# WU-CVGL/SIU3R

Hardware: AMD Instinct MI355X
Metric: image-pairs/sec @2x512^2 (SIU3R network forward incl. panoptic post-process) (higher is better)
Workload: dtype bf16x3 (fp32 activations, bf16 MFMA with hi/lo operand split; meets the 1e-3 parity bar)

## Files before the change

### siu3r_amd/csrc/gemm.hip

```cpp
#include <stdlib.h>

#include "common.h"
#include "gemm_epilogue.h"

int siu3r_gemm_dma_launch(const siu3r_gemm_params& p, int ni, void* stream);
int siu3r_gemm_dma_x3_launch(const siu3r_gemm_params& p, void* stream);
int siu3r_gemm_dma_mode(const siu3r_gemm_params& p);
int siu3r_gemm_dma_x3_mode(const siu3r_gemm_params& p);
int siu3r_gemm_pp_mode(const siu3r_gemm_params& p);
void siu3r_gemm_pp_name(const siu3r_gemm_params& p, int cfg, char* buf, int n);
int siu3r_gemm_pp_launch(const siu3r_gemm_params& p, int cfg, void* stream);
int siu3r_gemm_skinny_launch(const siu3r_gemm_params& p, void* stream);
int siu3r_gemm_skinny_path(const siu3r_gemm_params& p);
int siu3r_gemm_dma_kspl();
bool siu3r_gemm_pp_a_x3_ok(const siu3r_gemm_params& p);
bool siu3r_gemm_pp_c_x3_ok(const siu3r_gemm_params& p, int cfg);
static const bool g_disable_dma = getenv("SIU3R_GEMM_NO_DMA") != nullptr;
static const int g_narrow_max = getenv("SIU3R_GEMM_NARROW_MAX") ? atoi(getenv("SIU3R_GEMM_NARROW_MAX")) : 0x7fffffff;

namespace {

constexpr int BM = 128, BK = 64;
constexpr int A_TILE_BYTES = BM * BK * 2;

__device__ __forceinline__ int lds_off(int row, int chunk) {
  return row * 128 + ((chunk ^ ((row >> 1) & 7)) << 4);
}

template <int A_F32, int SPLIT, int NI>
struct Regs {
  float4 ra0[A_F32 ? 4 : 1], ra1[A_F32 ? 4 : 1];
  uint4 rab[A_F32 ? 1 : 4];
  uint4 rwh[2 * NI], rwl[SPLIT ? 2 * NI : 1];
};

template <int A_F32, int SPLIT, int NI, bool LNF = false>
__global__ __launch_bounds__(256) void gemm_kernel(const siu3r_gemm_params p) {
  constexpr int BN = 64 * NI;
  constexpr int B_TILE_BYTES = BN * BK * 2;
// ... 362 lines not shown
  const Cand& c = kCands[best];
  pl.tile_cfg = c.cfg;
  pl.bm = c.bm;
  pl.bn = c.bn;
  pl.splitk = best_s;
  pl.skinny_rows = best_skinny;
  if (c.cfg > 0 && best_skinny > 0) {
    siu3r_gemm_params q = p;
    q.m_main = p.m - best_skinny;
    pl.skinny_path = siu3r_gemm_skinny_path(q);
  }
  if (c.cfg < 0) {
    const int64_t tiles128 = (int64_t)((p.m + BM - 1) / BM) * ((p.n + 127) / 128) * Z;
    const bool narrow = (p.n <= 64) || (tiles128 < g_narrow_max && p.n > 64) || p.w_x3 != nullptr;
    pl.bn = narrow ? 64 : 128;
    if (!narrow || dma_mode < 0) pl.splitk = 1;
  }
  if (pl.splitk > 1) {
    const int64_t tiles = (int64_t)((p.m - pl.skinny_rows + pl.bm - 1) / pl.bm) * ((p.n + pl.bn - 1) / pl.bn) * Z;
    pl.ws_floats = tiles * pl.splitk * pl.bm * pl.bn;
    pl.counters = (int32_t)tiles;
  }
  auto tf = [](bool b) { return b ? "true" : "false"; };
  if (c.cfg > 0) {
    siu3r_gemm_pp_name(p, c.cfg, pl.kernel, sizeof(pl.kernel));
  } else if (x3 && dma_mode >= 0 && pl.bn == 64) {
    snprintf(pl.kernel, sizeof(pl.kernel), "siu3r_gemm_dma::gemm_dma_x3_kernel<%d, %s, %d, %s>", dma_mode, tf(dma_mode == 1 && p.relu_in), siu3r_gemm_dma_kspl(), tf(dma_mode == 0 && p.ln_stats));
  } else if (!x3 && !p.w_lo && dma_mode >= 0) {
    snprintf(pl.kernel, sizeof(pl.kernel), "siu3r_gemm_dma::gemm_dma_kernel<%d, %d, %s, %d, %s>", pl.bn / 64, dma_mode, tf(dma_mode == 1 && p.relu_in), siu3r_gemm_dma_kspl(), tf(dma_mode == 0 && p.ln_stats));
  } else {
    snprintf(pl.kernel, sizeof(pl.kernel), "gemm_kernel<%d, %d, %d%s>", p.a_dtype == SIU3R_F32 ? 1 : 0, p.w_lo ? 1 : 0, pl.bn / 64, p.ln_stats ? ", true" : "");
  }
}
}

static int validate_gemm(const siu3r_gemm_params& p) {
  SIU3R_CHECK(p.a && p.w_hi && (p.c || p.c_x3), "siu3r_gemm: null operand pointer");
  SIU3R_CHECK(p.m > 0 && p.n > 0 && p.k > 0, "siu3r_gemm: empty problem (m=%d n=%d k=%d)", p.m, p.n, p.k);
  SIU3R_CHECK(p.kpad % BK == 0 && p.kpad >= p.k, "siu3r_gemm: kpad=%d must be a multiple of 64 and >= k=%d", p.kpad, p.k);
  SIU3R_CHECK(p.a_dtype == SIU3R_BF16 || p.a_dtype == SIU3R_F32, "siu3r_gemm: bad a_dtype %d", p.a_dtype);
  SIU3R_CHECK(p.c_dtype == SIU3R_BF16 || p.c_dtype == SIU3R_F32, "siu3r_gemm: bad c_dtype %d", p.c_dtype);
  SIU3R_CHECK(!(p.w_lo && p.a_dtype != SIU3R_F32), "siu3r_gemm: bf16x3 mode needs fp32 activations");
  SIU3R_CHECK(p.a_mode >= 0 && p.a_mode <= 2, "siu3r_gemm: bad a_mode %d", p.a_mode);
  if (p.a_mode != 0) SIU3R_CHECK(p.oh > 0 && p.ow > 0 && p.ih > 0 && p.iw > 0 && (p.a_mode == 2 || (p.cin > 0 && p.kh > 0 && p.kw > 0 && p.stride > 0)),
                                 "siu3r_gemm: conv geometry must be positive (ih=%d iw=%d cin=%d kh=%d kw=%d stride=%d oh=%d ow=%d)", p.ih, p.iw, p.cin, p.kh, p.kw, p.stride, p.oh, p.ow);
  if (p.a_mode == 0) {
    SIU3R_CHECK(p.k % 8 == 0 && p.lda % 8 == 0, "siu3r_gemm: dense A needs k %% 8 == 0 and lda %% 8 == 0 (k=%d lda=%ld)", p.k, (long)p.lda);
  } else if (p.a_mode == 1) {
    SIU3R_CHECK(p.cin % 8 == 0 || (p.cin % 4 == 0 && p.w_x3 && p.a_dtype == SIU3R_F32 && !p.relu_in && !g_disable_dma),
                "siu3r_gemm: conv gather needs cin %% 8 == 0 (cin %% 4 == 0 for fp32 activations with w_x3) (cin=%d)", p.cin);
    SIU3R_CHECK(p.k == p.kh * p.kw * p.cin, "siu3r_gemm: conv k=%d != kh*kw*cin", p.k);
    SIU3R_CHECK(p.m % (p.oh * p.ow) == 0, "siu3r_gemm: conv m=%d not a multiple of oh*ow", p.m);
  } else {
    SIU3R_CHECK(p.a_dtype == SIU3R_F32 && p.k == 768 && p.ih == p.oh * 16 && p.iw == p.ow * 16,
                "siu3r_gemm: patchify mode needs fp32 NCHW input, k=768, H,W multiples of 16");
  }
  if (p.out_mode == 1) SIU3R_CHECK(p.n == p.up * p.up * p.cout && p.m % (p.ih * p.iw) == 0 && p.cout % 8 == 0, "siu3r_gemm: bad conv-transpose geometry (cout %% 8 == 0 required)");
  if (p.rope_cos) SIU3R_CHECK(p.rope_sin && p.rope_pos && p.rope_ncols % 64 == 0 && p.rope_ncols <= p.n && p.act == 0 && p.out_mode == 0,
                              "siu3r_gemm: bad RoPE epilogue arguments");
  if (p.up_src) SIU3R_CHECK(p.a_mode == 1 && p.out_mode == 0 && p.oh % 2 == 0 && p.ow % 2 == 0, "siu3r_gemm: up_src needs conv mode with even output size");
  if (p.ln_stats)
    SIU3R_CHECK(p.ln_c1 && p.ln_c2 && !p.bias && p.a_mode == 0 && p.ln_tiles == (p.k + 63) / 64 && p.ln_tiles <= 16 && !p.relu_in,
                "siu3r_gemm: folded LayerNorm needs c1/c2, no bias, dense A and ln_tiles == ceil(k/64) <= 16 (k=%d, ln_tiles=%d)", p.k, p.ln_tiles);
  if (p.stats_out) SIU3R_CHECK(p.out_mode == 0 && !p.up_src, "siu3r_gemm: stats_out needs a plain row-major output");
  if (p.c_aux) SIU3R_CHECK(p.out_mode == 0, "siu3r_gemm: c_aux needs a plain row-major output");
  if (p.splitk > 1)
    SIU3R_CHECK(p.sk_ws && p.sk_cnt && p.splitk <= 64 && p.splitk <= p.kpad / 64, "siu3r_gemm: split-K needs a workspace, zeroed counters and splitk <= kpad / 64 (splitk=%d)", p.splitk);
  SIU3R_CHECK(p.tile_cfg >= -1 && p.tile_cfg <= 3, "siu3r_gemm: bad tile_cfg %d", p.tile_cfg);
  if (p.bmod > 0) SIU3R_CHECK(p.batch > 0 && p.batch % p.bmod == 0, "siu3r_gemm: batch %d is not a multiple of bmod %d", p.batch, p.bmod);
  return 0;
}

extern "C" int siu3r_gemm_plan(const siu3r_gemm_params* pp, siu3r_gemm_plan_t* out) {
  SIU3R_CHECK(pp && out, "siu3r_gemm_plan: null argument");
  if (int rc = validate_gemm(*pp)) return rc;
  plan(*pp, *out);
  out->a_x3_ok = out->tile_cfg > 0 && siu3r_gemm_pp_a_x3_ok(*pp);
  out->c_x3_ok = out->tile_cfg > 0 && siu3r_gemm_pp_c_x3_ok(*pp, out->tile_cfg);
  return 0;
}

extern "C" int siu3r_gemm(const siu3r_gemm_params* pp, void* stream) {
  const siu3r_gemm_params& p = *pp;
  if (int rc = validate_gemm(p)) return rc;
  siu3r_gemm_plan_t pl;
  plan(p, pl);
  hipStream_t s = (hipStream_t)stream;
  SIU3R_CHECK(!p.a_x3 || (pl.tile_cfg > 0 && siu3r_gemm_pp_a_x3_ok(p)), "siu3r_gemm: a_x3 (pre-split A planes) needs a ping-pong plan, bf16x3 weights, dense A, "
              "k == kpad and lda / batch strides %% 32 == 0 (this block runs %s): query siu3r_gemm_plan_t.a_x3_ok first", pl.kernel);
  SIU3R_CHECK(!p.c_x3 || (pl.tile_cfg > 0 && siu3r_gemm_pp_c_x3_ok(p, pl.tile_cfg)), "siu3r_gemm: c_x3 (output planes) needs a ping-pong plan and the plain fp32 "
              "row-major output form with n %% 64 == 0, ldc / batch strides %% 32 == 0 (this block runs %s): query siu3r_gemm_plan_t.c_x3_ok first", pl.kernel);
  SIU3R_CHECK(p.c || p.c_x3, "siu3r_gemm: null output");
  siu3r_gemm_params q = p;
  q.splitk = pl.splitk;
  if (pl.splitk > 1) SIU3R_CHECK(p.sk_ws && p.sk_cnt && p.sk_ws_floats >= pl.ws_floats && p.sk_cnt_n >= pl.counters,
                                 "siu3r_gemm: split-K workspace too small (%ld floats / %d counters needed)", (long)pl.ws_floats, pl.counters);
  SIU3R_CHECK(!(p.splitk > 1 && pl.splitk != p.splitk), "siu3r_gemm: splitk=%d was requested but %s cannot split K for this problem (it would run %d slice(s)); "
              "request 0 / 1 or another tile_cfg", p.splitk, pl.kernel, pl.splitk);
  if (pl.tile_cfg > 0) {
    q.m_main = pl.skinny_rows > 0 ? p.m - pl.skinny_rows : 0;
    if (!(pl.skinny_rows > 0 && q.m_main == 0)) {
      const int rc = siu3r_gemm_pp_launch(q, pl.tile_cfg, stream);
      if (rc) return rc;
    }
    if (pl.skinny_rows > 0 && siu3r_gemm_skinny_path(q) != 1) {
      q.splitk = 0;
      return siu3r_gemm_skinny_launch(q, stream);
    }
    return 0;
  }
  return pl.bn == 64 ? launch<1>(q, s) : launch<2>(q, s);
}
```

### siu3r_amd/csrc/gemm_dma.hip

```cpp
#include <stdlib.h>

#include "common.h"
#include "gemm_epilogue.h"

namespace siu3r_gemm_dma {

constexpr int BM = 128, BK = 64, STAGES = 3;
#ifndef SIU3R_GEMM_PD_WIDE
#define SIU3R_GEMM_PD_WIDE 2
#endif
constexpr int A_TILE_BYTES = BM * BK * 2;
constexpr unsigned OOB = 0xffffff00u;
constexpr int RSRC_FLAGS = 0x00020000;

typedef __attribute__((address_space(3))) void* lds_ptr;
typedef __attribute__((ext_vector_type(4))) unsigned int u32x4;
typedef __attribute__((ext_vector_type(2))) short i16x2;

template <int NI, int MODE, bool RELU, int KSPL, bool LNF = false>
__global__ __launch_bounds__(256 * KSPL, NI == 1 ? 2 * KSPL : 1) void gemm_dma_kernel(const siu3r_gemm_params p) {
#if __HIP_DEVICE_COMPILE__
  constexpr int BN = 64 * NI;
  constexpr int B_TILE_BYTES = BN * BK * 2;
  constexpr int STAGE_BYTES = A_TILE_BYTES + B_TILE_BYTES;
// ... 337 lines not shown
  for (int kt = 0; kt < nkt; kt += 2) {
    tile_body(kt, st, fA0, fB0, fA1, fB1);
    st = (st + 1 == STAGES) ? 0 : st + 1;
    if (kt + 1 < nkt) {
      tile_body(kt + 1, st, fA1, fB1, fA0, fB0);
      st = (st + 1 == STAGES) ? 0 : st + 1;
    }
  }
#undef SIU3R_WAIT_FRAGS
  asm volatile("s_waitcnt vmcnt(0)" ::: "memory");
  stamp(4);

  if (dbg & 1) { if (acc[0][0][0] == 123.456f) ((float*)p.c)[0] = 1.f; return; }
  siu3r_epi::run<NI, KSPL, LNF>(p, acc, smem, tile_m, tile_n, z, t);
  if (trace && t == 0) {
    trace[6] = __builtin_readcyclecounter();
    asm volatile("s_waitcnt vmcnt(0)" ::: "memory");
    trace[7] = __builtin_readcyclecounter();
  }
#endif
}


template <int MODE, bool RELU, int KSPL, bool LNF = false>
__global__ __launch_bounds__(256 * KSPL, 2 * KSPL) void gemm_dma_x3_kernel(const siu3r_gemm_params p) {
#if __HIP_DEVICE_COMPILE__
  constexpr int BN = 64, BKE = 32;
  constexpr int B_TILE_BYTES = BN * 128;
  constexpr int STAGE_BYTES = A_TILE_BYTES + B_TILE_BYTES;
  constexpr int A_DMA = 4 / KSPL, W_DMA = 2 / KSPL, LP = A_DMA + W_DMA;
  constexpr int KSW = 2 / KSPL;
  static_assert(STAGES * STAGE_BYTES >= siu3r_epi::staging_bytes<1, KSPL>(), "epilogue staging must fit the ring");
  __shared__ __attribute__((aligned(128))) unsigned char smem[STAGES * STAGE_BYTES];

  const int t = threadIdx.x;
  const int lane = t & 63;
  const int wave = __builtin_amdgcn_readfirstlane(t >> 6);
  const int khalf = wave >> 2, wq = wave & 3;
  const int wm = wq >> 1, wn = wq & 1;
  const int l31 = lane & 31, lh = lane >> 5;

  const int M = p.m, N = p.n, K = p.k, kpad = p.kpad;
  const int tiles_m = (M + BM - 1) / BM, tiles_n = (N + BN - 1) / BN;
  const int xcd = (blockIdx.x + blockIdx.z) & 7, li = blockIdx.x >> 3;
  const int map_gx = p.map_gx;
  const int ry = xcd / map_gx, rx = xcd - ry * map_gx;
  const int lm = li / p.map_rn, ln = li - lm * p.map_rn;
  const int tile_m = ry * p.map_rm + lm, tile_n = rx * p.map_rn + ln;
  if (lm >= p.map_rm || tile_m >= tiles_m || tile_n >= tiles_n) return;
// ... 125 lines not shown
    unsigned char* dst = smem + stage * STAGE_BYTES + A_TILE_BYTES + (wave * W_DMA + i) * 1024;
    __builtin_amdgcn_raw_ptr_buffer_load_lds(rW, (lds_ptr)dst, 16, w_voff[i], (kbase + kt) * 128, 0, 0);
  };
  auto issue = [&](int kt, int stage) {
#pragma unroll
    for (int i = 0; i < A_DMA; ++i) issue_a(kt, stage, i);
#pragma unroll
    for (int i = 0; i < W_DMA; ++i) issue_w(kt, stage, i);
    if (MODE == 1) cursor_advance();
    if (MODE == 2) state_advance();
  };

  f32x16 acc[2][1];
#pragma unroll
  for (int i = 0; i < 2; ++i)
#pragma unroll
    for (int r = 0; r < 16; ++r) acc[i][0][r] = 0.f;

  const unsigned int lds_base = (unsigned int)(size_t)(__attribute__((address_space(3))) unsigned char*)smem;
  unsigned int offA[2], offB;
#pragma unroll
  for (int i = 0; i < 2; ++i) {
    const int row = wm * 64 + i * 32 + l31;
    offA[i] = row * 128 + ((((lh << 1)) ^ ((row >> 1) & 7)) << 4);
  }
  {
    const int row = wn * 32 + l31;
    offB = A_TILE_BYTES + row * 128 + ((lh ^ ((row >> 1) & 7)) << 4);
  }
  struct Frag {
    u32x4 a[2][2], bh, bl;
  };
  auto read_sub = [&](unsigned int sbase, int ks, Frag& f) {
#pragma unroll
    for (int i = 0; i < 2; ++i) {
      const unsigned int ad = (sbase + offA[i]) ^ (ks << 6);
      asm volatile("ds_read_b128 %0, %1" : "=v"(f.a[i][0]) : "v"(ad) : "memory");
      asm volatile("ds_read_b128 %0, %1 offset:0" : "=v"(f.a[i][1]) : "v"(ad ^ 16u) : "memory");
    }
    const unsigned int adb = (sbase + offB) ^ (ks << 5);
    asm volatile("ds_read_b128 %0, %1" : "=v"(f.bh) : "v"(adb) : "memory");
    asm volatile("ds_read_b128 %0, %1" : "=v"(f.bl) : "v"(adb ^ 64u) : "memory");
  };
  auto issue_tile_reads = [&](int stage, Frag (&f)[KSW]) {
    const unsigned int sbase = lds_base + stage * STAGE_BYTES;
#pragma unroll
    for (int j = 0; j < KSW; ++j) read_sub(sbase, khalf * KSW + j, f[j]);
  };
  auto split8 = [&](const u32x4& v0, const u32x4& v1, bf16x8& hi, bf16x8& lo) {
    unsigned int w[8] = {v0[0], v0[1], v0[2], v0[3], v1[0], v1[1], v1[2], v1[3]};
    union { u32x4 u; bf16x8 h; } H, L;
#pragma unroll
    for (int q = 0; q < 4; ++q) {
      unsigned int x0 = w[2 * q], x1 = w[2 * q + 1];
      if (RELU) {
        x0 = (x0 & 0x80000000u) ? 0u : x0;
        x1 = (x1 & 0x80000000u) ? 0u : x1;
      }
      const unsigned int h0 = x0 & 0xffff0000u, h1 = x1 & 0xffff0000u;
      const float l0 = __uint_as_float(x0) - __uint_as_float(h0), l1 = __uint_as_float(x1) - __uint_as_float(h1);
      H.u[q] = __builtin_amdgcn_perm(x1, x0, 0x07060302u);
// ... 17 lines not shown
#pragma unroll
        for (int i = 0; i < A_DMA; ++i) issue_a(kt_next, stage_next, i);
#pragma unroll
        for (int i = 0; i < W_DMA; ++i) issue_w(kt_next, stage_next, i);
      }
      if (j == KSW - 1 && kt + 1 < nkt) {
        if (kt_next >= 0) {
          if (LP == 6) asm volatile("s_waitcnt vmcnt(6)" ::: "memory");
          else asm volatile("s_waitcnt vmcnt(3)" ::: "memory");
        } else {
          asm volatile("s_waitcnt vmcnt(0)" ::: "memory");
        }
        __builtin_amdgcn_s_barrier();
        asm volatile("" ::: "memory");
        issue_tile_reads(stage_read, nf);
      }
      __builtin_amdgcn_sched_barrier(0);
      union { u32x4 u; bf16x8 h; } bh, bl;
      bh.u = f[j].bh;
      bl.u = f[j].bl;
#pragma unroll
      for (int i = 0; i < 2; ++i) {
        bf16x8 ah, al;
        split8(f[j].a[i][0], f[j].a[i][1], ah, al);
        acc[i][0] = __builtin_amdgcn_mfma_f32_32x32x16_bf16(al, bh.h, acc[i][0], 0, 0, 0);
        acc[i][0] = __builtin_amdgcn_mfma_f32_32x32x16_bf16(ah, bl.h, acc[i][0], 0, 0, 0);
        acc[i][0] = __builtin_amdgcn_mfma_f32_32x32x16_bf16(ah, bh.h, acc[i][0], 0, 0, 0);
      }
      if (KSW == 2 && kt_next >= 0 && j == 0) {
#pragma unroll
        for (int i = 0; i < A_DMA; ++i) issue_a(kt_next, stage_next, i);
#pragma unroll
        for (int i = 0; i < W_DMA; ++i) issue_w(kt_next, stage_next, i);
      }
      __builtin_amdgcn_sched_barrier(0);
    }
    if (MODE == 1 && kt_next >= 0) cursor_advance();
    if (MODE == 2 && kt_next >= 0) state_advance();
  };

  for (int q = 0; q < kbase; ++q) {
    if (MODE == 1) cursor_advance();
    if (MODE == 2) state_advance();
  }
  issue(0, 0);
  if (nkt > 1) issue(1, 1);
  if (nkt > 1) {
    if (LP == 6) asm volatile("s_waitcnt vmcnt(6)" ::: "memory");
    else asm volatile("s_waitcnt vmcnt(3)" ::: "memory");
  } else {
    asm volatile("s_waitcnt vmcnt(0)" ::: "memory");
  }
  __builtin_amdgcn_s_barrier();
  asm volatile("" ::: "memory");
  Frag f0[KSW], f1[KSW];
  issue_tile_reads(0, f0);
  int st = 0;
  for (int kt = 0; kt < nkt; kt += 2) {
    tile_body(kt, st, f0, f1);
    st = (st + 1 == STAGES) ? 0 : st + 1;
    if (kt + 1 < nkt) {
      tile_body(kt + 1, st, f1, f0);
      st = (st + 1 == STAGES) ? 0 : st + 1;
    }
  }
#undef SIU3R_X3_WAIT
  asm volatile("s_waitcnt vmcnt(0)" ::: "memory");
  siu3r_epi::run<1, KSPL, LNF>(p, acc, smem, tile_m, tile_n, z, t);
#endif
}

}

int siu3r_gemm_dma_mode(const siu3r_gemm_params& p) {
  const int64_t lim = 0xfffff000ll;
  if (p.w_lo || p.a_dtype != SIU3R_BF16 || p.a_mode == 2) return -1;
  if ((int64_t)p.n * p.kpad * 2 >= lim) return -1;
  if (p.a_mode == 0) return (((int64_t)(p.m - 1) * p.lda + p.k) * 2 >= lim || p.relu_in) ? -1 : 0;
  const int64_t img = (int64_t)(p.m / (p.oh * p.ow)) * p.ih * p.iw * p.cin * 2 + (int64_t)(p.pad * p.iw + p.pad) * p.cin * 2;
  if (img >= lim) return -1;
  const int mode = (p.cin % 64 == 0 && p.kh * p.kw <= 32 && p.kpad == p.k) ? 1 : 2;
  return (mode == 2 && p.relu_in) ? -1 : mode;
}
int siu3r_gemm_dma_x3_mode(const siu3r_gemm_params& p) {
  const int64_t lim = 0xfffff000ll;
  if (!p.w_x3 || p.a_dtype != SIU3R_F32 || (int64_t)p.n * p.kpad * 4 >= lim) return -1;
  if (p.a_mode == 0) return (((int64_t)(p.m - 1) * p.lda + p.k) * 4 >= lim || p.relu_in) ? -1 : 0;
  if (p.a_mode != 1) return -1;
  const int64_t img = (int64_t)(p.m / (p.oh * p.ow)) * p.ih * p.iw * p.cin * 4 + (int64_t)(p.pad * p.iw + p.pad) * p.cin * 4;
  if (img >= lim || p.cin % 4 != 0) return -1;
  if (p.cin % 32 == 0 && p.kh * p.kw <= 31) return 1;
  return p.relu_in ? -1 : 2;
}

int siu3r_gemm_dma_kspl() {
  static const bool no_ksplit = getenv("SIU3R_GEMM_NO_KSPLIT") != nullptr;
  return no_ksplit ? 1 : 2;
}

int siu3r_gemm_dma_launch(const siu3r_gemm_params& p, int ni, void* stream) {
  using namespace siu3r_gemm_dma;
  const int64_t lim = 0xfffff000ll;
  int mode;
  if ((int64_t)p.n * p.kpad * 2 >= lim) return 1;
  if (p.a_mode == 0) {
    mode = 0;
    if (((int64_t)(p.m - 1) * p.lda + p.k) * 2 >= lim || p.relu_in) return 1;
  } else {
    const int64_t img = (int64_t)(p.m / (p.oh * p.ow)) * p.ih * p.iw * p.cin * 2 + (int64_t)(p.pad * p.iw + p.pad) * p.cin * 2;
    if (img >= lim) return 1;
    mode = (p.cin % 64 == 0 && p.kh * p.kw <= 32 && p.kpad == p.k) ? 1 : 2;
    if (mode == 2 && p.relu_in) return 1;
  }
  const int tiles = 8 * p.map_rm * p.map_rn;
  dim3 grid(tiles, p.splitk > 1 ? p.splitk : 1, p.batch > 0 ? p.batch : 1);
// ... 20 lines not shown
}

int siu3r_gemm_dma_x3_launch(const siu3r_gemm_params& p, void* stream) {
  using namespace siu3r_gemm_dma;
  const int64_t lim = 0xfffff000ll;
  if (!p.w_x3 || p.a_dtype != SIU3R_F32 || (int64_t)p.n * p.kpad * 4 >= lim) return 1;
  int mode;
  if (p.a_mode == 0) {
    mode = 0;
    if (((int64_t)(p.m - 1) * p.lda + p.k) * 4 >= lim || p.relu_in) return 1;
  } else if (p.a_mode == 1) {
    const int64_t img = (int64_t)(p.m / (p.oh * p.ow)) * p.ih * p.iw * p.cin * 4 + (int64_t)(p.pad * p.iw + p.pad) * p.cin * 4;
    if (img >= lim || p.cin % 4 != 0) return 1;
    if (p.cin % 32 == 0 && p.kh * p.kw <= 31) mode = 1;
    else if (!p.relu_in) mode = 2;
    else return 1;
  } else {
    return 1;
  }
  const int tiles = 8 * p.map_rm * p.map_rn;
  dim3 grid(tiles, p.splitk > 1 ? p.splitk : 1, p.batch > 0 ? p.batch : 1);
  hipStream_t s = (hipStream_t)stream;
  const bool no_ksplit = siu3r_gemm_dma_kspl() == 1;
  if (mode == 0 && p.ln_stats) {
    if (no_ksplit) hipLaunchKernelGGL((gemm_dma_x3_kernel<0, false, 1, true>), grid, dim3(256), 0, s, p);
    else hipLaunchKernelGGL((gemm_dma_x3_kernel<0, false, 2, true>), grid, dim3(512), 0, s, p);
  } else if (no_ksplit) {
    if (mode == 0) hipLaunchKernelGGL((gemm_dma_x3_kernel<0, false, 1>), grid, dim3(256), 0, s, p);
    else if (mode == 2) hipLaunchKernelGGL((gemm_dma_x3_kernel<2, false, 1>), grid, dim3(256), 0, s, p);
    else if (p.relu_in) hipLaunchKernelGGL((gemm_dma_x3_kernel<1, true, 1>), grid, dim3(256), 0, s, p);
    else hipLaunchKernelGGL((gemm_dma_x3_kernel<1, false, 1>), grid, dim3(256), 0, s, p);
  } else {
    if (mode == 0) hipLaunchKernelGGL((gemm_dma_x3_kernel<0, false, 2>), grid, dim3(512), 0, s, p);
    else if (mode == 2) hipLaunchKernelGGL((gemm_dma_x3_kernel<2, false, 2>), grid, dim3(512), 0, s, p);
    else if (p.relu_in) hipLaunchKernelGGL((gemm_dma_x3_kernel<1, true, 2>), grid, dim3(512), 0, s, p);
    else hipLaunchKernelGGL((gemm_dma_x3_kernel<1, false, 2>), grid, dim3(512), 0, s, p);
  }
  SIU3R_LAUNCH_CHECK("siu3r_gemm(dma x3)");
  return 0;
}
```

### siu3r_amd/csrc/gemm_epilogue.h

```cpp
#pragma once
#include "common.h"

namespace siu3r_epi {

__device__ __forceinline__ float gelu_fast(float x) {
  const float ax = fabsf(x);
  float q = 4.30638e-5f * 0.125f;
  q = q * ax + 2.765672e-4f * 0.17677669529663687f;
  q = q * ax + 1.520143e-4f * 0.25f;
  q = q * ax + 9.2705272e-3f * 0.35355339059327373f;
  q = q * ax + 4.22820123e-2f * 0.5f;
  q = q * ax + 7.05230784e-2f * 0.70710678118654752f;
  q = q * ax + 1.0f;
  q *= q;
  q *= q;
  q *= q;
  q *= q;
  const float e = 1.0f - __builtin_amdgcn_rcpf(q);
  return 0.5f * (ax * e + x);
}

template <int NI, int KSPL = 1>
constexpr int staging_bytes() { return 128 * (64 * NI + 4) * 4 + 2048; }

template <int NI, int KSPL = 1, bool LNF = false>
__device__ __forceinline__ void run(const siu3r_gemm_params& p, f32x16 (&acc)[2][NI], unsigned char* smem, int tile_m,
                                    int tile_n, int z, int t) {
  constexpr int BN = 64 * NI, BM = 128;
  constexpr int LDC = BN + 4;
  constexpr int CHUNKS = BN / 8;
  constexpr int RPP = 256 * KSPL / CHUNKS;
  constexpr int NTASK = BM / RPP;
  constexpr int G = NTASK < 4 ? NTASK : 4, NG = NTASK / G;
  float* cs = (float*)smem;
  const int lane = t & 63, wave = (t >> 6) & 3, kh = t >> 8;
  const int wm = wave >> 1, wn = wave & 1;
  const int l31 = lane & 31, lh = lane >> 5;
  unsigned char* Cb = (unsigned char*)p.c;
  const unsigned char* Rb = (const unsigned char*)p.residual;
  const siu3r_zoff zof = siu3r_batch_offsets(p, z);
  const int64_t c_boff = zof.c, r_boff = zof.r;
  const float* biasp = p.bias ? p.bias + zof.bias : nullptr;
  constexpr bool ln = LNF;
  const float* c1p = ln ? p.ln_c1 + zof.bias : nullptr;
  const float* c2p = ln ? p.ln_c2 + zof.bias : nullptr;
  float* s_ln = cs + BM * LDC;
  float* s_c1 = s_ln + 2 * BM;
  const int c_esz = p.c_dtype == SIU3R_F32 ? 4 : 2;
// ... 308 lines not shown
        float s1 = 0.f;
#pragma unroll
        for (int e = 0; e < 8; ++e) s1 += e < nv ? v[e] : 0.f;
        s1 += __shfl_xor(s1, 1);
        s1 += __shfl_xor(s1, 2);
        s1 += __shfl_xor(s1, 4);
        const float mean = s1 / (float)max(n64, 1);
        float s2 = 0.f;
#pragma unroll
        for (int e = 0; e < 8; ++e) {
          const float d = v[e] - mean;
          s2 += e < nv ? d * d : 0.f;
        }
        s2 += __shfl_xor(s2, 1);
        s2 += __shfl_xor(s2, 2);
        s2 += __shfl_xor(s2, 4);
        if ((chunk & 7) == 0 && n64 > 0) {
          const int64_t row = (int64_t)zof.zo * p.st_sz + (int64_t)zof.zi * p.st_sz_i + (int64_t)m * p.st_ldm;
          ((float2*)p.stats_out)[row * ((N + 63) >> 6) + (n0 >> 6)] = make_float2(mean, s2);
        }
        if (!col_ok) continue;
      }
      const int64_t cidx = c_boff + oidx;
      if (full && (((uintptr_t)Cb + cidx * c_esz) & 15) == 0) {
        f32x8 o;
#pragma unroll
        for (int e = 0; e < 8; ++e) o.v[e] = v[e];
        store8_from_f32(Cb, p.c_dtype, cidx, o);
        if (p.c_aux) store8_from_f32(p.c_aux, SIU3R_BF16, cidx, o);
      } else {
        _Pragma("unroll") for (int e = 0; e < 8; ++e)
          if (e < nv) {
            store_from_f32(Cb, p.c_dtype, cidx + e, v[e]);
            if (p.c_aux) store_from_f32(p.c_aux, SIU3R_BF16, cidx + e, v[e]);
          }
      }
    }
  }
}

}
```

### siu3r_amd/model.py

```python
from __future__ import annotations

import functools
import math
from typing import Dict, List, Optional, Sequence

import os

import torch
import torch.nn.functional as F

from . import ops
from .ops import ACT_GELU, ACT_NONE, ACT_RELU
from .gaussians_types import Gaussians
from . import postprocess as pp

ENC_HEADS, DEC_HEADS = 16, 12
ADAPTER_IDX = (5, 11, 17, 23)
DPT_HOOKS = (0, 6, 9, 12)


class _Weights:

    def __init__(self, sd: Dict[str, torch.Tensor], device, split: bool):
        self.sd, self.dev, self.split = sd, device, split
# ... 273 lines not shown
        e = self.encode_begin(images, K)
        self.encode_blocks(e, 0, self.enc_depth)
        return self.encode_end(e)

    def _ctx_positions(self, B, V, h, w):
        key = ("ctxpos", B, V, h, w)
        c = self.ctx.cache
        if key not in c:
            pv = self._positions(B * V, h, w).view(B, V, h * w + 1, 2)
            c[key] = torch.stack([torch.cat([pv[:, j] for j in range(V) if j != i], dim=1) for i in range(1, V)], dim=1).flatten(0, 1).contiguous()
        return c[key]

    def decode_begin(self, enc):
        ctx = self.ctx
        B, V, H, W, N = enc["dims"]
        h, w = H // 16, W // 16
        x, pos = enc["x"], enc["pos"]
        f = ctx.ln("backbone.enc_norm", x, 1e-6, out_dtype=torch.float32)
        merged = ctx.fold and V == 2
        g = torch.empty((B, V, N + 1, self.dec_embed_dim), dtype=torch.float32, device=ctx.dev)
        gs = [g] + [torch.empty_like(g) for _ in range(self.dec_depth)]
        gstat = [ops.RowStats(t) for t in gs] if merged else None
        gb16 = [None if (ctx.split or not merged) else torch.empty(t.shape, dtype=torch.bfloat16, device=ctx.dev) for t in gs]
        ops.linear(f, ctx.w.linear("backbone.decoder_embed"), out=g.view(B * V * (N + 1), -1), stats_out=gstat[0] if merged else None,
                   aux_out=None if gb16[0] is None else gb16[0].view(B * V * (N + 1), -1))
        fv = f.view(B, V, N + 1, -1)
        pv = pos.view(B, V, N + 1, 2)
        pos0 = pv[:, 0].contiguous()
        if V == 2:
            pos_rest, mem0_pos, memr_pos = pv[:, 1].contiguous(), pv[:, 1].contiguous(), pos0
        else:
            pos_rest = pv[:, 1:].reshape(B * (V - 1), N + 1, 2).contiguous()
            mem0_pos = pv[:, 1:].reshape(B, (V - 1) * (N + 1), 2).contiguous()
            memr_pos = self._ctx_positions(B, V, h, w)
        return dict(enc=enc, fv=fv, g=gs, gstat=gstat, gb16=gb16, pos0=pos0, pos_rest=pos_rest, mem0_pos=mem0_pos, memr_pos=memr_pos, rope=enc["rope"],
                    merged=merged)

    def decode_layer_merged(self, d, i):
        ctx = self.ctx
        B, V, H, W, N = d["enc"]["dims"]
        x, xs, xb = d["g"][i], d["gstat"][i], d["gb16"][i]
        Cc = x.shape[-1]
        hd = Cc // DEC_HEADS
        rope, pos = d["rope"], d["enc"]["pos"]
        sides = [f"backbone.dec_blocks.{i}", f"backbone.dec_blocks2.{i}"]
        W_ = ctx.w
        grp = lambda tag, build: W_.group(f"dec{i}.{tag}", build, sides)
        A = lambda t, tb: t if ctx.split else tb
        if _DEC_QKVX:
            other = {sides[0]: sides[1], sides[1]: sides[0]}
            build = lambda q: ops.cat_packed([W_.linear_ln_rows(q + ".attn.qkv", (0, 2 * Cc), q + ".norm1"),
                                              W_.linear_ln(other[q] + ".cross_attn.projk", other[q] + ".norm_y"),
                                              W_.linear_ln_rows(q + ".attn.qkv", (2 * Cc, 3 * Cc), q + ".norm1"),
                                              W_.linear_ln(other[q] + ".cross_attn.projv", other[q] + ".norm_y")])
            pj_buf = torch.empty((B, V, N + 1, 5 * Cc), dtype=ctx.act, device=x.device)
            pj = pj_buf.view(B * V, N + 1, 5, DEC_HEADS, hd)
            att = dict(heads=DEC_HEADS, head_dim=hd, scale=hd ** -0.5, split3=ctx.split)
            kvp = ops.Planes(pj_buf, storage=pj_buf) if (ctx.split and _KV_PLANES and ops.attention(pj[:, :, 0], pj[:, :, 1], pj[:, :, 3], dry_run=True, **att)) else None
            ops.linear_grouped(A(x, xb), grp("qkvx", build), ln=xs, rope=(rope[0], rope[1], pos, 3 * Cc), out=pj_buf, planes_out=kvp, planes_from_col=Cc)
            kvp = kvp is not None and kvp.valid
            self_qkv = (pj[:, :, 0], pj[:, :, 1], pj[:, :, 3])
        else:
            pj, kvp = None, False
            att = dict(heads=DEC_HEADS, head_dim=hd, scale=hd ** -0.5, split3=ctx.split)
            qkv = ops.linear_grouped(A(x, xb), grp("qkv", lambda q: W_.linear_ln(q + ".attn.qkv", q + ".norm1")), out_dtype=ctx.act, ln=xs,
                                     rope=(rope[0], rope[1], pos, 2 * Cc)).view(B * V, N + 1, 3, DEC_HEADS, hd)
            self_qkv = (qkv[:, :, 0], qkv[:, :, 1], qkv[:, :, 2])

        def attend(tag, wname, qkv_, res, S_out, **kw):
            xo, so, bo = S_out
            wp = grp(tag, lambda q: W_.linear(q + wname))
            a4 = torch.empty((B, V, N + 1, Cc), dtype=ctx.act, device=x.device)
            ap = _feeds_planes("dec_attn", ctx, a4, lambda t: ops.linear_grouped(t, wp, residual=res, out=xo, stats_out=so, aux_out=bo, dry_run=True))
            ops.attention(*qkv_, out=a4.view(B * V, N + 1, Cc), planes_out=ap, planes_only=True, **att, **kw)
            ops.linear_grouped(a4, wp, residual=res, out=xo, stats_out=so, aux_out=bo, a_planes=ap)

        S1 = x1, s1, b1 = self._new_stream(x)
        attend("proj", ".attn.proj", self_qkv, x, S1, kv_planes=kvp)
        qq = ops.linear_grouped(A(x1, b1), grp("projq", lambda q: W_.linear_ln(q + ".cross_attn.projq", q + ".norm2")), out_dtype=ctx.act, ln=s1,
                                rope=(rope[0], rope[1], pos, Cc)).view(B * V, N + 1, DEC_HEADS, hd)
        S2 = x2, s2, b2 = self._new_stream(x)
        if pj is not None:
            attend("xproj", ".cross_attn.proj", (qq, pj[:, :, 2], pj[:, :, 4]), x1, S2, kv_bxor=1, kv_planes=kvp)
        else:
            kv = ops.linear_grouped(A(x, xb), grp("projkv", lambda q: W_.linear_ln([q + ".cross_attn.projk", q + ".cross_attn.projv"], q + ".norm_y")),
                                    out_dtype=ctx.act, ln=xs, flip=True, rope=(rope[0], rope[1], pos, Cc)).view(B * V, N + 1, 2, DEC_HEADS, hd)
            attend("xproj", ".cross_attn.proj", (qq, kv[:, :, 0], kv[:, :, 1]), x1, S2)
        w1, w2 = grp("fc1", lambda q: W_.linear_ln(q + ".mlp.fc1", q + ".norm3")), grp("fc2", lambda q: W_.linear(q + ".mlp.fc2"))
        out2 = dict(residual=x2, out=d["g"][i + 1], stats_out=d["gstat"][i + 1], aux_out=d["gb16"][i + 1])
        h = torch.empty((B, V, N + 1, w1.n), dtype=ctx.act, device=x.device)
        hp = _feeds_planes("dec_fc", ctx, h, lambda t: ops.linear_grouped(t, w2, dry_run=True, **out2))
        ops.linear_grouped(A(x2, b2), w1, act=ACT_GELU, ln=s2, out=h, planes_out=hp, planes_only=True)
        ops.linear_grouped(h, w2, a_planes=hp, **out2)

    def decode_side(self, d, i, side):
        B, V, H, W, N = d["enc"]["dims"]
        g, g_next, rope = d["g"][i], d["g"][i + 1], d["rope"]
        if side == 0:
            mem0 = g[:, 1] if V == 2 else g[:, 1:].reshape(B, (V - 1) * (N + 1), -1)
            self._dec_block(f"backbone.dec_blocks.{i}", g[:, 0], mem0, d["pos0"], d["mem0_pos"], rope, out=g_next[:, 0])
            return
        if V == 2:
            xr, memr, outr = g[:, 1], g[:, 0], g_next[:, 1]
        else:
            xr = g[:, 1:].reshape(B * (V - 1), N + 1, -1)
            memr = torch.stack([torch.cat([g[:, j] for j in range(V) if j != v], dim=1) for v in range(1, V)], dim=1).flatten(0, 1)
            outr = g_next[0, 1:] if B == 1 else None
        r = self._dec_block(f"backbone.dec_blocks2.{i}", xr, memr, d["pos_rest"], d["memr_pos"], rope, out=outr)
        if outr is None:
            g_next[:, 1:].copy_(r.view(B, V - 1, N + 1, -1))

    def decode_end(self, d):
        B, V, H, W, N = d["enc"]["dims"]
        layers = [d["fv"]] + d["g"][1:]
        last = self.ctx.ln("backbone.dec_norm", layers[-1].reshape(B * V, N + 1, -1), 1e-6, out_dtype=torch.float32)
# ... 571 lines not shown
    def forward_nhwc(self, feats_nhwc: Sequence[torch.Tensor], B: int, T: int, lat1=None):
        mask_features, ms = self._pixel_decoder(feats_nhwc, lat1)
        class_logits, mask_cl, all_masks, inters = self._decoder(ms, mask_features, B, T)
        out = VideoMask2FormerForVideoSegmentationOutput(
            loss=None, class_queries_logits=class_logits,
            masks_queries_logits=mask_cl.permute(0, 4, 1, 2, 3),
            auxiliary_logits=None, attentions=None, word_embeddings=None,
        )
        out["_masks_channel_last"] = mask_cl
        out["_mask_features"], out["_ms"] = mask_features, ms
        return out

    def forward(self, multi_scale_feat: List[torch.Tensor], word_embeddings=None, mask_labels=None, class_labels=None, **kw):
        assert word_embeddings is None and mask_labels is None and class_labels is None, "inference path only"
        B, T = multi_scale_feat[0].shape[:2]
        feats = [f.flatten(0, 1).permute(0, 2, 3, 1).contiguous() for f in multi_scale_feat]
        return self.forward_nhwc(feats, B, T)

    __call__ = forward


_KV_PLANES = not os.environ.get("SIU3R_NO_KV_PLANES")
_CONV_PLANES = not os.environ.get("SIU3R_NO_CONV_PLANES")
_PRODUCER_PLANES_SITES = ("enc_attn", "dec_attn", "dec_fc", "pts_resize", "pts_fusion", "ext_msd", "ext_dw")
_PRODUCER_PLANES_DEFAULT = ("enc_attn", "pts_resize", "pts_fusion")
_PRODUCER_PLANES = frozenset(s_ for s_ in os.environ.get("SIU3R_PRODUCER_PLANES", ",".join(_PRODUCER_PLANES_DEFAULT)).split(",") if s_)
assert _PRODUCER_PLANES <= set(_PRODUCER_PLANES_SITES), _PRODUCER_PLANES


def _feeds_planes(site: str, ctx, like: torch.Tensor, plan) -> Optional[ops.Planes]:
    if site not in _PRODUCER_PLANES or ops._NO_PRESPLIT or not ctx.split or like.dtype != torch.float32:
        return None
    return ops.Planes(like, storage=like) if plan(like).a_x3_ok else None


_DEC_QKVX = not os.environ.get("SIU3R_NO_DEC_QKVX")
_HEAD_PAIRS = os.environ.get("SIU3R_NO_HEAD_PAIRS", "0") != "1"
_DEC_PER_LAYER = os.environ.get("SIU3R_DEC_PER_LAYER", "0") == "1"

_MAIN, _SEG, _DEC, _H0, _H1 = range(5)


@functools.lru_cache(maxsize=None)
def _schedule(paired: bool, merged: bool, dec_depth: int, pipelined: bool):
    steps = [("run", _MAIN, "enc_begin"), ("wait", _SEG, _MAIN), ("run", _SEG, "spm")]
    for k in range(len(ADAPTER_IDX)):
        steps += [("run", _MAIN, f"enc{k}"), ("wait", _SEG, _MAIN), ("run", _SEG, f"int{k}")]
    steps += [("run", _SEG, "seg"), ("after_seg", _SEG, None), ("run", _MAIN, "dec_pre")]
    if merged:
        steps += [("run", _MAIN, f"dec{i}") for i in range(dec_depth)] if _DEC_PER_LAYER else [("run", _MAIN, "dec_all")]
    for i in range(0 if merged else dec_depth):
        steps += [("wait", _DEC, _MAIN), ("run", _MAIN, f"decA{i}"), ("run", _DEC, f"decB{i}"), ("wait", _MAIN, _DEC)]
    steps += [("run", _MAIN, "dec_post"), ("wait", _H0, _MAIN), ("wait", _H1, _MAIN), ("wait", _SEG, _MAIN)]
    if paired:
        steps += [("run", _H0, "gs"), ("run", _H1 if pipelined else _MAIN, "pts")]
    else:
# ... 331 lines not shown
```

Before: 56.94.

## Let the bf16x3 LDS-DMA GEMM consume and emit pre-split hi/lo planes

Adds APS/X3O template variants to the bf16x3 LDS-DMA kernel. With APS it reads activations that were already split into bf16 hi/lo planes, which removes the in-kernel split. With X3O its epilogue writes hi/lo output planes for the next consumer. Plan queries now report a_x3_ok/c_x3_ok for this kernel, and the decoder's dec_attn and dec_fc producer-plane sites are on by default. The dec_stream site is wired but off by default. The cost is extra plane writes and more template instantiations, and the planes contract requires 128-byte alignment.

```diff
diff --git a/siu3r_amd/csrc/gemm.hip b/siu3r_amd/csrc/gemm.hip
--- a/siu3r_amd/csrc/gemm.hip
+++ b/siu3r_amd/csrc/gemm.hip
@@ -15,6 +15,8 @@
 int siu3r_gemm_dma_kspl();
 bool siu3r_gemm_pp_a_x3_ok(const siu3r_gemm_params& p);
 bool siu3r_gemm_pp_c_x3_ok(const siu3r_gemm_params& p, int cfg);
+bool siu3r_gemm_dma_a_x3_ok(const siu3r_gemm_params& p);
+bool siu3r_gemm_dma_c_x3_ok(const siu3r_gemm_params& p);
 static const bool g_disable_dma = getenv("SIU3R_GEMM_NO_DMA") != nullptr;
 static const int g_narrow_max = getenv("SIU3R_GEMM_NARROW_MAX") ? atoi(getenv("SIU3R_GEMM_NARROW_MAX")) : 0x7fffffff;
 
@@ -423,15 +425,29 @@
     pl.counters = (int32_t)tiles;
   }
   auto tf = [](bool b) { return b ? "true" : "false"; };
+  const bool chosen = (p.tile_cfg ? p.tile_cfg : g_tile_default) == 0;
+  const bool aps = chosen && p.a_x3 && siu3r_gemm_dma_a_x3_ok(p), x3o = chosen && p.c_x3 && siu3r_gemm_dma_c_x3_ok(p);
   if (c.cfg > 0) {
     siu3r_gemm_pp_name(p, c.cfg, pl.kernel, sizeof(pl.kernel));
   } else if (x3 && dma_mode >= 0 && pl.bn == 64) {
-    snprintf(pl.kernel, sizeof(pl.kernel), "siu3r_gemm_dma::gemm_dma_x3_kernel<%d, %s, %d, %s>", dma_mode, tf(dma_mode == 1 && p.relu_in), siu3r_gemm_dma_kspl(), tf(dma_mode == 0 && p.ln_stats));
+    snprintf(pl.kernel, sizeof(pl.kernel), "siu3r_gemm_dma::gemm_dma_x3_kernel<%d, %s, %d, %s%s>", dma_mode, tf(dma_mode == 1 && p.relu_in), siu3r_gemm_dma_kspl(), tf(dma_mode == 0 && p.ln_stats),
+             !(dma_mode == 0 && chosen) ? "" : x3o ? (aps ? ", true, true" : ", false, true") : aps ? ", true" : "");
   } else if (!x3 && !p.w_lo && dma_mode >= 0) {
     snprintf(pl.kernel, sizeof(pl.kernel), "siu3r_gemm_dma::gemm_dma_kernel<%d, %d, %s, %d, %s>", pl.bn / 64, dma_mode, tf(dma_mode == 1 && p.relu_in), siu3r_gemm_dma_kspl(), tf(dma_mode == 0 && p.ln_stats));
   } else {
     snprintf(pl.kernel, sizeof(pl.kernel), "gemm_kernel<%d, %d, %d%s>", p.a_dtype == SIU3R_F32 ? 1 : 0, p.w_lo ? 1 : 0, pl.bn / 64, p.ln_stats ? ", true" : "");
   }
+}
+
+bool plan_is_dma_x3(const siu3r_gemm_params& p, const siu3r_gemm_plan_t& pl) {
+  const bool chosen = (p.tile_cfg ? p.tile_cfg : g_tile_default) == 0;
+  return chosen && pl.tile_cfg < 0 && pl.bn == 64 && !g_disable_dma && p.w_x3 && p.a_dtype == SIU3R_F32 && siu3r_gemm_dma_x3_mode(p) >= 0;
+}
+bool plan_a_x3_ok(const siu3r_gemm_params& p, const siu3r_gemm_plan_t& pl) {
+  return pl.tile_cfg > 0 ? siu3r_gemm_pp_a_x3_ok(p) : plan_is_dma_x3(p, pl) && siu3r_gemm_dma_a_x3_ok(p);
+}
+bool plan_c_x3_ok(const siu3r_gemm_params& p, const siu3r_gemm_plan_t& pl) {
+  return pl.tile_cfg > 0 ? siu3r_gemm_pp_c_x3_ok(p, pl.tile_cfg) : plan_is_dma_x3(p, pl) && siu3r_gemm_dma_c_x3_ok(p);
 }
 }
 
@@ -476,8 +492,8 @@
   SIU3R_CHECK(pp && out, "siu3r_gemm_plan: null argument");
   if (int rc = validate_gemm(*pp)) return rc;
   plan(*pp, *out);
-  out->a_x3_ok = out->tile_cfg > 0 && siu3r_gemm_pp_a_x3_ok(*pp);
-  out->c_x3_ok = out->tile_cfg > 0 && siu3r_gemm_pp_c_x3_ok(*pp, out->tile_cfg);
+  out->a_x3_ok = plan_a_x3_ok(*pp, *out);
+  out->c_x3_ok = plan_c_x3_ok(*pp, *out);
   return 0;
 }
 
@@ -487,10 +503,12 @@
   siu3r_gemm_plan_t pl;
   plan(p, pl);
   hipStream_t s = (hipStream_t)stream;
-  SIU3R_CHECK(!p.a_x3 || (pl.tile_cfg > 0 && siu3r_gemm_pp_a_x3_ok(p)), "siu3r_gemm: a_x3 (pre-split A planes) needs a ping-pong plan, bf16x3 weights, dense A, "
-              "k == kpad and lda / batch strides %% 32 == 0 (this block runs %s): query siu3r_gemm_plan_t.a_x3_ok first", pl.kernel);
-  SIU3R_CHECK(!p.c_x3 || (pl.tile_cfg > 0 && siu3r_gemm_pp_c_x3_ok(p, pl.tile_cfg)), "siu3r_gemm: c_x3 (output planes) needs a ping-pong plan and the plain fp32 "
-              "row-major output form with n %% 64 == 0, ldc / batch strides %% 32 == 0 (this block runs %s): query siu3r_gemm_plan_t.c_x3_ok first", pl.kernel);
+  SIU3R_CHECK(!p.a_x3 || plan_a_x3_ok(p, pl), "siu3r_gemm: a_x3 (pre-split A planes) needs a ping-pong plan, bf16x3 weights, dense A, "
+              "k == kpad and lda / batch strides %% 32 == 0 -- or the bf16x3 LDS-DMA kernel where the launcher chose it (tile_cfg 0): dense A, "
+              "planes on a 128-byte line (this block runs %s): query siu3r_gemm_plan_t.a_x3_ok first", pl.kernel);
+  SIU3R_CHECK(!p.c_x3 || plan_c_x3_ok(p, pl), "siu3r_gemm: c_x3 (output planes) needs a ping-pong plan and the plain fp32 "
+              "row-major output form with n %% 64 == 0, ldc / batch strides %% 32 == 0 -- or the bf16x3 LDS-DMA kernel where the launcher chose it "
+              "(tile_cfg 0): dense A, planes on a 128-byte line (this block runs %s): query siu3r_gemm_plan_t.c_x3_ok first", pl.kernel);
   SIU3R_CHECK(p.c || p.c_x3, "siu3r_gemm: null output");
   siu3r_gemm_params q = p;
   q.splitk = pl.splitk;
diff --git a/siu3r_amd/csrc/gemm_dma.hip b/siu3r_amd/csrc/gemm_dma.hip
--- a/siu3r_amd/csrc/gemm_dma.hip
+++ b/siu3r_amd/csrc/gemm_dma.hip
@@ -383,9 +383,10 @@
 }
 
 
-template <int MODE, bool RELU, int KSPL, bool LNF = false>
+template <int MODE, bool RELU, int KSPL, bool LNF = false, bool APS = false, bool X3O = false>
 __global__ __launch_bounds__(256 * KSPL, 2 * KSPL) void gemm_dma_x3_kernel(const siu3r_gemm_params p) {
 #if __HIP_DEVICE_COMPILE__
+  static_assert(!(APS || X3O) || (MODE == 0 && !RELU), "pre-split operands: dense rows only");
   constexpr int BN = 64, BKE = 32;
   constexpr int B_TILE_BYTES = BN * 128;
   constexpr int STAGE_BYTES = A_TILE_BYTES + B_TILE_BYTES;
@@ -557,7 +558,7 @@
 #pragma unroll
   for (int i = 0; i < 2; ++i) {
     const int row = wm * 64 + i * 32 + l31;
-    offA[i] = row * 128 + ((((lh << 1)) ^ ((row >> 1) & 7)) << 4);
+    offA[i] = row * 128 + ((((APS ? lh : lh << 1)) ^ ((row >> 1) & 7)) << 4);
   }
   {
     const int row = wn * 32 + l31;
@@ -569,9 +570,9 @@
   auto read_sub = [&](unsigned int sbase, int ks, Frag& f) {
 #pragma unroll
     for (int i = 0; i < 2; ++i) {
-      const unsigned int ad = (sbase + offA[i]) ^ (ks << 6);
+      const unsigned int ad = (sbase + offA[i]) ^ (ks << (APS ? 5 : 6));
       asm volatile("ds_read_b128 %0, %1" : "=v"(f.a[i][0]) : "v"(ad) : "memory");
-      asm volatile("ds_read_b128 %0, %1 offset:0" : "=v"(f.a[i][1]) : "v"(ad ^ 16u) : "memory");
+      asm volatile("ds_read_b128 %0, %1 offset:0" : "=v"(f.a[i][1]) : "v"(ad ^ (APS ? 64u : 16u)) : "memory");
     }
     const unsigned int adb = (sbase + offB) ^ (ks << 5);
     asm volatile("ds_read_b128 %0, %1" : "=v"(f.bh) : "v"(adb) : "memory");
@@ -635,7 +636,15 @@
 #pragma unroll
       for (int i = 0; i < 2; ++i) {
         bf16x8 ah, al;
-        split8(f[j].a[i][0], f[j].a[i][1], ah, al);
+        if (APS) {
+          union { u32x4 u; bf16x8 h; } H, L;
+          H.u = f[j].a[i][0];
+          L.u = f[j].a[i][1];
+          ah = H.h;
+          al = L.h;
+        } else {
+          split8(f[j].a[i][0], f[j].a[i][1], ah, al);
+        }
         acc[i][0] = __builtin_amdgcn_mfma_f32_32x32x16_bf16(al, bh.h, acc[i][0], 0, 0, 0);
         acc[i][0] = __builtin_amdgcn_mfma_f32_32x32x16_bf16(ah, bl.h, acc[i][0], 0, 0, 0);
         acc[i][0] = __builtin_amdgcn_mfma_f32_32x32x16_bf16(ah, bh.h, acc[i][0], 0, 0, 0);
@@ -679,8 +688,14 @@
   }
 #undef SIU3R_X3_WAIT
   asm volatile("s_waitcnt vmcnt(0)" ::: "memory");
-  siu3r_epi::run<1, KSPL, LNF>(p, acc, smem, tile_m, tile_n, z, t);
+  siu3r_epi::run<1, KSPL, LNF, X3O>(p, acc, smem, tile_m, tile_n, z, t);
 #endif
+}
+
+template <bool LNF, bool APS, bool X3O>
+static void launch_x3_planes(const siu3r_gemm_params& p, dim3 grid, bool no_ksplit, hipStream_t s) {
+  if (no_ksplit) gemm_dma_x3_kernel<0, false, 1, LNF, APS, X3O><<<grid, dim3(256), 0, s>>>(p);
+  else gemm_dma_x3_kernel<0, false, 2, LNF, APS, X3O><<<grid, dim3(512), 0, s>>>(p);
 }
 
 }
@@ -704,6 +719,14 @@
   if (img >= lim || p.cin % 4 != 0) return -1;
   if (p.cin % 32 == 0 && p.kh * p.kw <= 31) return 1;
   return p.relu_in ? -1 : 2;
+}
+bool siu3r_gemm_dma_a_x3_ok(const siu3r_gemm_params& p) {
+  return siu3r_gemm_dma_x3_mode(p) == 0 && p.k == p.kpad && p.lda % 32 == 0 && p.sa % 32 == 0 && p.sa_i % 32 == 0 && ((uintptr_t)p.a % 128) == 0;
+}
+bool siu3r_gemm_dma_c_x3_ok(const siu3r_gemm_params& p) {
+  return siu3r_gemm_dma_x3_mode(p) == 0 && p.c_x3 && ((uintptr_t)p.c_x3 % 128) == 0 && ((uintptr_t)p.c % 16) == 0 && p.out_mode == 0 &&
+         p.c_dtype == SIU3R_F32 && p.n % 64 == 0 && p.ldc % 32 == 0 && p.sc % 32 == 0 && p.sc_i % 32 == 0 && p.c_x3_col0 >= 0 &&
+         p.c_x3_col0 % 64 == 0;
 }
 
 int siu3r_gemm_dma_kspl() {
@@ -770,7 +793,19 @@
   dim3 grid(tiles, p.splitk > 1 ? p.splitk : 1, p.batch > 0 ? p.batch : 1);
   hipStream_t s = (hipStream_t)stream;
   const bool no_ksplit = siu3r_gemm_dma_kspl() == 1;
-  if (mode == 0 && p.ln_stats) {
+  if (p.a_x3 || p.c_x3) {
+    if ((p.a_x3 && !siu3r_gemm_dma_a_x3_ok(p)) || (p.c_x3 && !siu3r_gemm_dma_c_x3_ok(p))) {
+      siu3r_set_error("siu3r_gemm(dma x3): a_x3 / c_x3 outside the LDS-DMA kernel's planes contract");
+      return -1;
+    }
+    const int v = (p.ln_stats ? 4 : 0) | (p.a_x3 ? 2 : 0) | (p.c_x3 ? 1 : 0);
+    if (v == 1) launch_x3_planes<false, false, true>(p, grid, no_ksplit, s);
+    else if (v == 2) launch_x3_planes<false, true, false>(p, grid, no_ksplit, s);
+    else if (v == 3) launch_x3_planes<false, true, true>(p, grid, no_ksplit, s);
+    else if (v == 5) launch_x3_planes<true, false, true>(p, grid, no_ksplit, s);
+    else if (v == 6) launch_x3_planes<true, true, false>(p, grid, no_ksplit, s);
+    else launch_x3_planes<true, true, true>(p, grid, no_ksplit, s);
+  } else if (mode == 0 && p.ln_stats) {
     if (no_ksplit) hipLaunchKernelGGL((gemm_dma_x3_kernel<0, false, 1, true>), grid, dim3(256), 0, s, p);
     else hipLaunchKernelGGL((gemm_dma_x3_kernel<0, false, 2, true>), grid, dim3(512), 0, s, p);
   } else if (no_ksplit) {
diff --git a/siu3r_amd/csrc/gemm_epilogue.h b/siu3r_amd/csrc/gemm_epilogue.h
--- a/siu3r_amd/csrc/gemm_epilogue.h
+++ b/siu3r_amd/csrc/gemm_epilogue.h
@@ -23,7 +23,7 @@
 template <int NI, int KSPL = 1>
 constexpr int staging_bytes() { return 128 * (64 * NI + 4) * 4 + 2048; }
 
-template <int NI, int KSPL = 1, bool LNF = false>
+template <int NI, int KSPL = 1, bool LNF = false, bool X3O = false>
 __device__ __forceinline__ void run(const siu3r_gemm_params& p, f32x16 (&acc)[2][NI], unsigned char* smem, int tile_m,
                                     int tile_n, int z, int t) {
   constexpr int BN = 64 * NI, BM = 128;
@@ -378,11 +378,23 @@
         if (!col_ok) continue;
       }
       const int64_t cidx = c_boff + oidx;
+      bool st_c = true;
+      if (X3O && p.c_x3) {
+        const bool x3o = n0 >= p.c_x3_col0;
+        st_c = Cb != nullptr && !(x3o && p.c_x3 == p.c);
+        if (x3o) {
+          uint4 hi, lo;
+          split_trunc_bf16x8(v, hi, lo);
+          unsigned char* seg = (unsigned char*)p.c_x3 + (cidx - (n0 & 31)) * 4 + ((n0 & 31) >> 3) * 16;
+          *(uint4*)seg = hi;
+          *(uint4*)(seg + 64) = lo;
+        }
+      }
       if (full && (((uintptr_t)Cb + cidx * c_esz) & 15) == 0) {
         f32x8 o;
 #pragma unroll
         for (int e = 0; e < 8; ++e) o.v[e] = v[e];
-        store8_from_f32(Cb, p.c_dtype, cidx, o);
+        if (st_c) store8_from_f32(Cb, p.c_dtype, cidx, o);
         if (p.c_aux) store8_from_f32(p.c_aux, SIU3R_BF16, cidx, o);
       } else {
         _Pragma("unroll") for (int e = 0; e < 8; ++e)
diff --git a/siu3r_amd/model.py b/siu3r_amd/model.py
--- a/siu3r_amd/model.py
+++ b/siu3r_amd/model.py
@@ -319,6 +319,7 @@
         gs = [g] + [torch.empty_like(g) for _ in range(self.dec_depth)]
         gstat = [ops.RowStats(t) for t in gs] if merged else None
         gb16 = [None if (ctx.split or not merged) else torch.empty(t.shape, dtype=torch.bfloat16, device=ctx.dev) for t in gs]
+        gplanes = [_stream_planes(ctx, t) if merged and 0 < j < self.dec_depth else None for j, t in enumerate(gs)]
         ops.linear(f, ctx.w.linear("backbone.decoder_embed"), out=g.view(B * V * (N + 1), -1), stats_out=gstat[0] if merged else None,
                    aux_out=None if gb16[0] is None else gb16[0].view(B * V * (N + 1), -1))
         fv = f.view(B, V, N + 1, -1)
@@ -330,13 +331,13 @@
             pos_rest = pv[:, 1:].reshape(B * (V - 1), N + 1, 2).contiguous()
             mem0_pos = pv[:, 1:].reshape(B, (V - 1) * (N + 1), 2).contiguous()
             memr_pos = self._ctx_positions(B, V, h, w)
-        return dict(enc=enc, fv=fv, g=gs, gstat=gstat, gb16=gb16, pos0=pos0, pos_rest=pos_rest, mem0_pos=mem0_pos, memr_pos=memr_pos, rope=enc["rope"],
+        return dict(enc=enc, fv=fv, g=gs, gstat=gstat, gb16=gb16, gplanes=gplanes, pos0=pos0, pos_rest=pos_rest, mem0_pos=mem0_pos, memr_pos=memr_pos, rope=enc["rope"],
                     merged=merged)
 
     def decode_layer_merged(self, d, i):
         ctx = self.ctx
         B, V, H, W, N = d["enc"]["dims"]
-        x, xs, xb = d["g"][i], d["gstat"][i], d["gb16"][i]
+        x, xs, xb, xp = d["g"][i], d["gstat"][i], d["gb16"][i], d["gplanes"][i]
         Cc = x.shape[-1]
         hd = Cc // DEC_HEADS
         rope, pos = d["rope"], d["enc"]["pos"]
@@ -354,29 +355,29 @@
             pj = pj_buf.view(B * V, N + 1, 5, DEC_HEADS, hd)
             att = dict(heads=DEC_HEADS, head_dim=hd, scale=hd ** -0.5, split3=ctx.split)
             kvp = ops.Planes(pj_buf, storage=pj_buf) if (ctx.split and _KV_PLANES and ops.attention(pj[:, :, 0], pj[:, :, 1], pj[:, :, 3], dry_run=True, **att)) else None
-            ops.linear_grouped(A(x, xb), grp("qkvx", build), ln=xs, rope=(rope[0], rope[1], pos, 3 * Cc), out=pj_buf, planes_out=kvp, planes_from_col=Cc)
+            ops.linear_grouped(A(x, xb), grp("qkvx", build), ln=xs, rope=(rope[0], rope[1], pos, 3 * Cc), out=pj_buf, a_planes=xp, planes_out=kvp, planes_from_col=Cc)
             kvp = kvp is not None and kvp.valid
             self_qkv = (pj[:, :, 0], pj[:, :, 1], pj[:, :, 3])
         else:
             pj, kvp = None, False
             att = dict(heads=DEC_HEADS, head_dim=hd, scale=hd ** -0.5, split3=ctx.split)
-            qkv = ops.linear_grouped(A(x, xb), grp("qkv", lambda q: W_.linear_ln(q + ".attn.qkv", q + ".norm1")), out_dtype=ctx.act, ln=xs,
+            qkv = ops.linear_grouped(A(x, xb), grp("qkv", lambda q: W_.linear_ln(q + ".attn.qkv", q + ".norm1")), out_dtype=ctx.act, ln=xs, a_planes=xp,
                                      rope=(rope[0], rope[1], pos, 2 * Cc)).view(B * V, N + 1, 3, DEC_HEADS, hd)
             self_qkv = (qkv[:, :, 0], qkv[:, :, 1], qkv[:, :, 2])
 
         def attend(tag, wname, qkv_, res, S_out, **kw):
-            xo, so, bo = S_out
+            xo, so, bo, po = S_out
             wp = grp(tag, lambda q: W_.linear(q + wname))
             a4 = torch.empty((B, V, N + 1, Cc), dtype=ctx.act, device=x.device)
-            ap = _feeds_planes("dec_attn", ctx, a4, lambda t: ops.linear_grouped(t, wp, residual=res, out=xo, stats_out=so, aux_out=bo, dry_run=True))
+            ap = _feeds_planes("dec_attn", ctx, a4, lambda t: ops.linear_grouped(t, wp, residual=res, out=xo, stats_out=so, aux_out=bo, planes_out=po, dry_run=True))
             ops.attention(*qkv_, out=a4.view(B * V, N + 1, Cc), planes_out=ap, planes_only=True, **att, **kw)
-            ops.linear_grouped(a4, wp, residual=res, out=xo, stats_out=so, aux_out=bo, a_planes=ap)
-
-        S1 = x1, s1, b1 = self._new_stream(x)
+            ops.linear_grouped(a4, wp, residual=res, out=xo, stats_out=so, aux_out=bo, a_planes=ap, planes_out=po)
+
+        S1 = x1, s1, b1, xp1 = (*self._new_stream(x), _stream_planes(ctx, x))
         attend("proj", ".attn.proj", self_qkv, x, S1, kv_planes=kvp)
-        qq = ops.linear_grouped(A(x1, b1), grp("projq", lambda q: W_.linear_ln(q + ".cross_attn.projq", q + ".norm2")), out_dtype=ctx.act, ln=s1,
+        qq = ops.linear_grouped(A(x1, b1), grp("projq", lambda q: W_.linear_ln(q + ".cross_attn.projq", q + ".norm2")), out_dtype=ctx.act, ln=s1, a_planes=xp1,
                                 rope=(rope[0], rope[1], pos, Cc)).view(B * V, N + 1, DEC_HEADS, hd)
-        S2 = x2, s2, b2 = self._new_stream(x)
+        S2 = x2, s2, b2, xp2 = (*self._new_stream(x), _stream_planes(ctx, x))
         if pj is not None:
             attend("xproj", ".cross_attn.proj", (qq, pj[:, :, 2], pj[:, :, 4]), x1, S2, kv_bxor=1, kv_planes=kvp)
         else:
@@ -384,10 +385,10 @@
                                     out_dtype=ctx.act, ln=xs, flip=True, rope=(rope[0], rope[1], pos, Cc)).view(B * V, N + 1, 2, DEC_HEADS, hd)
             attend("xproj", ".cross_attn.proj", (qq, kv[:, :, 0], kv[:, :, 1]), x1, S2)
         w1, w2 = grp("fc1", lambda q: W_.linear_ln(q + ".mlp.fc1", q + ".norm3")), grp("fc2", lambda q: W_.linear(q + ".mlp.fc2"))
-        out2 = dict(residual=x2, out=d["g"][i + 1], stats_out=d["gstat"][i + 1], aux_out=d["gb16"][i + 1])
+        out2 = dict(residual=x2, out=d["g"][i + 1], stats_out=d["gstat"][i + 1], aux_out=d["gb16"][i + 1], planes_out=d["gplanes"][i + 1])
         h = torch.empty((B, V, N + 1, w1.n), dtype=ctx.act, device=x.device)
         hp = _feeds_planes("dec_fc", ctx, h, lambda t: ops.linear_grouped(t, w2, dry_run=True, **out2))
-        ops.linear_grouped(A(x2, b2), w1, act=ACT_GELU, ln=s2, out=h, planes_out=hp, planes_only=True)
+        ops.linear_grouped(A(x2, b2), w1, act=ACT_GELU, ln=s2, a_planes=xp2, out=h, planes_out=hp, planes_only=True)
         ops.linear_grouped(h, w2, a_planes=hp, **out2)
 
     def decode_side(self, d, i, side):
@@ -1005,8 +1006,8 @@
 
 _KV_PLANES = not os.environ.get("SIU3R_NO_KV_PLANES")
 _CONV_PLANES = not os.environ.get("SIU3R_NO_CONV_PLANES")
-_PRODUCER_PLANES_SITES = ("enc_attn", "dec_attn", "dec_fc", "pts_resize", "pts_fusion", "ext_msd", "ext_dw")
-_PRODUCER_PLANES_DEFAULT = ("enc_attn", "pts_resize", "pts_fusion")
+_PRODUCER_PLANES_SITES = ("enc_attn", "dec_attn", "dec_fc", "dec_stream", "pts_resize", "pts_fusion", "ext_msd", "ext_dw")
+_PRODUCER_PLANES_DEFAULT = ("enc_attn", "dec_attn", "dec_fc", "pts_resize", "pts_fusion")
 _PRODUCER_PLANES = frozenset(s_ for s_ in os.environ.get("SIU3R_PRODUCER_PLANES", ",".join(_PRODUCER_PLANES_DEFAULT)).split(",") if s_)
 assert _PRODUCER_PLANES <= set(_PRODUCER_PLANES_SITES), _PRODUCER_PLANES
 
@@ -1015,6 +1016,12 @@
     if site not in _PRODUCER_PLANES or ops._NO_PRESPLIT or not ctx.split or like.dtype != torch.float32:
         return None
     return ops.Planes(like, storage=like) if plan(like).a_x3_ok else None
+
+
+def _stream_planes(ctx, like: torch.Tensor) -> Optional[ops.Planes]:
+    if "dec_stream" not in _PRODUCER_PLANES or ops._NO_PRESPLIT or not ctx.split or like.dtype != torch.float32:
+        return None
+    return ops.Planes(like)
 
 
 _DEC_QKVX = not os.environ.get("SIU3R_NO_DEC_QKVX")
```

Result: no change. 57.07, median of 6 (+0.2%).
